# I2S9/dexterous-rl-manipulation

Measured on AMD Instinct MI355X. Metric: env-steps/sec @4096 envs/GPU, 1/2/4/8 MI355X; %HBM roofline step kernel, higher is better.
Workload: dtype bf16 MFMA (f32 acc) + f32/f64 env; 1 GPU; config_easy.json PG iteration: fused actor-MLP(256,256) rollout of 200 env steps x 4096 envs + critic fwd + GAE + adv-norm + PPO-clip / value heads + backward + Adam (1 epoch x 1 minibatch: ratio == 1, an A2C-style step); learner=pg, envs_per_gpu=4096, global_envs=4096, horizon=200, parallelism=dp1, world_size=1, ranks_per_gpu=1, overlap_comm=False, reserve_cus=0, reuse_h2=True

## Files before the change

### dexterous-rl-manipulation_amd/csrc/dxrl_mfma.h

```cpp
#pragma once
#include <hip/hip_runtime.h>
#include <stdint.h>

namespace dxrl {

typedef __bf16 bf16;
typedef bf16 bf16x8 __attribute__((ext_vector_type(8)));
typedef float f32x16 __attribute__((ext_vector_type(16)));
typedef bf16 bf16x4 __attribute__((ext_vector_type(4)));
typedef __attribute__((address_space(3))) bf16x4 lds_bf16x4;
typedef __attribute__((address_space(3))) bf16 lds_bf16;

__device__ __forceinline__ bf16x8 zero8() {
    bf16x8 z;
#pragma unroll
    for (int j = 0; j < 8; ++j) z[j] = (bf16)0.0f;
    return z;
}

__device__ __forceinline__ f32x16 mfma32(const bf16x8& a, const bf16x8& b, const f32x16& c) {
    return __builtin_amdgcn_mfma_f32_32x32x16_bf16(a, b, c, 0, 0, 0);
}

typedef float f32x4 __attribute__((ext_vector_type(4)));
__device__ __forceinline__ f32x4 mfma16(const bf16x8& a, const bf16x8& b, const f32x4& c) {
    return __builtin_amdgcn_mfma_f32_16x16x32_bf16(a, b, c, 0, 0, 0);
}

__device__ __forceinline__ bf16 to_bf16(float x) { return (bf16)x; }
__device__ __forceinline__ float from_bf16(bf16 x) { return (float)x; }

__device__ __forceinline__ int acc_row(int reg, int lane) { return (reg & 3) + 8 * (reg >> 2) + 4 * (lane >> 5); }

__device__ __forceinline__ bf16x8 load_frag(const bf16* base, int64_t ld, int64_t row, int64_t rows_valid, int k) {
    if (row < rows_valid) return *reinterpret_cast<const bf16x8*>(base + row * ld + k);
    bf16x8 z;
#pragma unroll
    for (int j = 0; j < 8; ++j) z[j] = (bf16)0.0f;
    return z;
}
// ... 71 lines not shown
```

### dexterous-rl-manipulation_amd/csrc/dxrl_pg_fused.hip

```cpp
#include "dxrl_gemm.h"
#include "dxrl_pg.h"

#include <stdio.h>
#include <stdlib.h>

#include <vector>

using namespace dxrl;
using namespace dxrl::pg;

namespace dxrl {
namespace {

constexpr float kLog2PiF = 1.8378770664093453f;
constexpr int kXp = kIn + 8;
constexpr int kHp = kH + 8;
constexpr int kDp = kOut + 8;

template <int kTR>
struct TileLds {
    static constexpr int kOffX = 0;
    static constexpr int kOffH1 = kOffX + kTR * kXp;
    static constexpr int kOffH2 = kOffH1 + kTR * kHp;
    static constexpr int kOffD = kOffH2 + kTR * kHp;
    static constexpr int kElems = kOffD + kTR * kDp;
    static_assert(kElems * 2 * (128 / kTR) == 163840, "one CU's 160 KiB of LDS per 128 samples");
};

// ... 16 lines not shown
    const bf16* X;
    const bf16 *W1, *W2, *W3, *W2T, *W3T;
    const bf16* W3rm;
    const float* b2;
    const float* b3;
    const float* logstd;
    const float* act;
    const float* logp_old;
    const float* adv;
    const float* ret;
    const double* stats;
    float sc, clip_eps, vf2;
    float* v_out;
    bf16* h1_out;
    bf16* dh2_out;
    const bf16* h2_in;
    bf16* h2_out;
    float* part;
    double* loss;
    int loss_rows;
    unsigned long long* stamps;
};

__device__ __forceinline__ void glds_x4(const void* src, const void* lds_dst) {
    const uint32_t lds_addr =
        __builtin_amdgcn_readfirstlane((uint32_t)(uintptr_t)(__attribute__((address_space(3))) const char*)lds_dst);
    uint32_t keep;
    asm volatile("s_mov_b32 %0, m0\n\ts_mov_b32 m0, %2\n\ts_nop 0\n\tglobal_load_lds_dwordx4 %1, off\n\ts_mov_b32 m0, %0"
                 : "=&s"(keep)
                 : "v"(src), "s"(lds_addr)
                 : "memory");
}

__device__ __forceinline__ void zero_acc(f32x16& a) {
#pragma unroll
    for (int q = 0; q < 16; ++q) a[q] = 0.0f;
}

struct NoHook {
    __device__ void operator()() const {}
};
struct NoKHook {
    __device__ void operator()(int) const {}
};
template <int KS>
struct WPre {
    static constexpr int kD = KS < 8 ? KS : 8;
    bf16x8 wf[kD];
    const gbf16x8* wp;
};
template <int KS>
__device__ __forceinline__ void w_prefetch(WPre<KS>& w, const bf16* W, int kst, int ft0, int lane) {
    w.wp = (const gbf16x8*)W + (int64_t)ft0 * kst * 64 + lane;
#pragma unroll
    for (int k = 0; k < WPre<KS>::kD; ++k) w.wf[k] = w.wp[64 * k];
}
template <int KS, int kLda, int MT, typename Hook = NoHook>
__device__ __forceinline__ void fwd_run(WPre<KS>& w, const bf16* A, f32x16 (&acc)[MT], int lane, Hook hook = Hook{},
                                        bool no_mfma = false) {
    const int r = lane & 31, h = lane >> 5;
    constexpr int kD = WPre<KS>::kD;
#pragma unroll
    for (int mt = 0; mt < MT; ++mt) zero_acc(acc[mt]);
    const bf16* ap = A + r * kLda + 8 * h;
    bf16x8 bq[2][MT];
#pragma unroll
    for (int mt = 0; mt < MT; ++mt) bq[0][mt] = *reinterpret_cast<const bf16x8*>(ap + 32 * mt * kLda);
#pragma unroll
    for (int k = 0; k < KS; ++k) {
        if (k + 1 < KS) {
#pragma unroll
            for (int mt = 0; mt < MT; ++mt)
                bq[(k + 1) & 1][mt] = *reinterpret_cast<const bf16x8*>(ap + 32 * mt * kLda + 16 * (k + 1));
        }
        const bf16x8 a = w.wf[k % kD];
        if (k + kD < KS) w.wf[k % kD] = w.wp[64 * (k + kD)];
        if (k + kD == KS) hook();
        __builtin_amdgcn_sched_barrier(0);
#pragma unroll
        for (int mt = 0; mt < MT; ++mt)
            if (!no_mfma) acc[mt] = mfma32(a, bq[k & 1][mt], acc[mt]);
        __builtin_amdgcn_sched_barrier(0);
    }
}
template <int KS, int kLda, int MT, typename Hook = NoHook>
__device__ __forceinline__ void fwd_tiles(const bf16* __restrict__ W, int kst, int ft0, const bf16* A,
                                          f32x16 (&acc)[MT], int lane, Hook hook = Hook{}, bool no_mfma = false) {
    WPre<KS> w;
    w_prefetch(w, W, kst, ft0, lane);
    fwd_run<KS, kLda, MT>(w, A, acc, lane, hook, no_mfma);
}

template <int KS, int kLda, int MT, typename Epi, typename KHook = NoKHook, typename THook = NoKHook>
__device__ __forceinline__ void fwd_pipe_w(const bf16x8 (&wf)[KS], const bf16* A, int lane, Epi& epi,
                                           bool no_mfma = false, KHook khook = KHook{}, THook thook = THook{}) {
    static_assert(KS >= 4 && KS % 4 == 0, "pair schedule assumes KS in {4, 8, 16, ...}");
    const int r = lane & 31, h = lane >> 5;
    constexpr int kPairsPerK = KS >= 8 ? 1 : 8 / KS;
    constexpr int kKPerPair = KS >= 8 ? KS / 8 : 1;
// ... 22 lines not shown
                for (int q = 0; q < kPairsPerK; ++q) epi(prev, mt - 1, (k / kKPerPair) * kPairsPerK + q);
            }
            khook(sidx);
            __builtin_amdgcn_sched_barrier(0);
        }
        prev = acc;
    }
    epi.prime(MT - 1);
#pragma unroll
    for (int q = 0; q < 8; ++q) {
        epi(prev, MT - 1, q);
        thook(q);
    }
}
template <int KS, int kLda, int MT, typename Epi, typename Hook = NoHook, typename KHook = NoKHook,
          typename THook = NoKHook>
__device__ __forceinline__ void fwd_pipe(WPre<KS>& w, const bf16* A, int lane, Epi& epi, Hook hook = Hook{},
                                         bool no_mfma = false, KHook khook = KHook{}, THook thook = THook{}) {
    constexpr int kD = WPre<KS>::kD;
    bf16x8 wf[KS];
#pragma unroll
    for (int k = 0; k < kD; ++k) wf[k] = w.wf[k];
#pragma unroll
    for (int k = kD; k < KS; ++k) wf[k] = w.wp[64 * k];
    hook();
    fwd_pipe_w<KS, kLda, MT>(wf, A, lane, epi, no_mfma, khook, thook);
}

struct EpiTanh {
    bf16* H;
    int f0;
    int r;
    const float* bk;
    bf16x4 v;
    __device__ void prime(int) {}
    __device__ __forceinline__ void operator()(const f32x16& acc, int mt, int p) {
        const int g = p >> 1, u = 2 * (p & 1);
        const f32x2 b = bk ? f32x2{bk[4 * g + u], bk[4 * g + u + 1]} : f32x2{0.0f, 0.0f};
        const f32x2 t = tanh_pre2(f32x2{acc[4 * g + u], acc[4 * g + u + 1]}, b);
        v[u] = to_bf16(t.x);
        v[u + 1] = to_bf16(t.y);
        if (u == 2) *reinterpret_cast<bf16x4*>(H + (32 * mt + r) * kHp + f0 + 8 * g) = v;
    }
};
struct EpiTanhB {
    bf16* H;
    int f0;
// ... 66 lines not shown
template <int MT>
__device__ __forceinline__ void gate_store(const f32x16 (&acc)[MT], const bf16x4 (&ys)[4][MT], int ft, bf16* Y,
                                           int lane) {
    const int r = lane & 31, h = lane >> 5;
#pragma unroll
    for (int g = 0; g < 4; ++g) {
        const int f0 = 32 * ft + 8 * g + 4 * h;
#pragma unroll
        for (int mt = 0; mt < MT; ++mt) {
            const bf16x4 y = ys[g][mt];
            bf16x4 v;
#pragma unroll
            for (int u = 0; u < 4; u += 2) {
                const f32x2 t = tanh_gate2(f32x2{acc[mt][4 * g + u], acc[mt][4 * g + u + 1]},
                                           f32x2{from_bf16(y[u]), from_bf16(y[u + 1])});
                v[u] = to_bf16(t.x);
                v[u + 1] = to_bf16(t.y);
            }
            *reinterpret_cast<bf16x4*>(Y + (32 * mt + r) * kHp + f0) = v;
        }
    }
}

template <int kThreads, int kTR>
__device__ __forceinline__ void copy_tile_out_n(const bf16* T, bf16* out, int64_t ld, int64_t m0, int64_t rows,
                                                int t, int diag) {
    constexpr int kChunks = kTR * (kH / 8);
    static_assert(kChunks % kThreads == 0, "whole chunks per thread");
    if (diag & 1) return;
    asm volatile("" : "+v"(t));
#pragma unroll
    for (int u = 0; u < kChunks / kThreads; ++u) {
        const int c = t + kThreads * u, row = c >> 5, col = 8 * (c & 31);
        const int64_t m = m0 + row;
        const bf16x8 v = *reinterpret_cast<const bf16x8*>(T + row * kHp + col);
        if (m < rows) *(__attribute__((address_space(1))) bf16x8*)(out + m * ld + col) = v;
    }
}

__device__ __forceinline__ void store_dh2(bf16* dst, const bf16x8& v) { *(__attribute__((address_space(1))) bf16x8*)dst = v; }

template <typename T>
__device__ __forceinline__ T* opaque(T* ptr) {
    asm volatile("" : "+s"(ptr));
    return ptr;
}

#ifndef DXRL_L2_PIPE
#define DXRL_L2_PIPE 1
#endif
#ifndef DXRL_DH2_IN_DH1
#define DXRL_DH2_IN_DH1 1
#endif
#ifndef DXRL_CRITIC_HEAD16
#define DXRL_CRITIC_HEAD16 1
#endif
#ifndef DXRL_ACTOR_HEAD16
#define DXRL_ACTOR_HEAD16 1
#endif
#ifndef DXRL_HEAD_PF
#define DXRL_HEAD_PF 1
#endif
#ifndef DXRL_FWD_RESIDENT_W
// ... 64 lines not shown
        for (int q = 0; q < 4; ++q) {
            acc3[j][0][q] = acc3[j][1][q] = 0.0f;
#pragma unroll
            for (int ri = 0; ri < 2; ++ri)
#pragma unroll
                for (int ci = 0; ci < 3; ++ci) acc1[j][ri][ci][q] = 0.0f;
        }
    float dls[8], db3[8];
#pragma unroll
    for (int j = 0; j < 8; ++j) dls[j] = db3[j] = 0.0f;
    float db2 = 0.0f;
    float lsum[4] = {0.0f, 0.0f, 0.0f, 0.0f};

    const auto uniform_f64 = [](double v) {
        const uint64_t u = __double_as_longlong(v);
        const uint32_t lo = __builtin_amdgcn_readfirstlane((uint32_t)u), hi = __builtin_amdgcn_readfirstlane((uint32_t)(u >> 32));
        return __longlong_as_double((long long)(((uint64_t)hi << 32) | lo));
    };
    const double adv_mean = uniform_f64(kTrain && actor ? p.stats[2] : 0.0);
    const double adv_inv = uniform_f64(kTrain && actor ? 1.0 / (p.stats[4] + 1e-8) : 1.0);

    constexpr int kXU = kTR * (kIn / 8) / kFThreads;
    bf16x8 xr[kXU];
    auto fetch_x = [&](int64_t tile) {
        int t = tid;
        asm volatile("" : "+v"(t));
#pragma unroll
        for (int u = 0; u < kXU; ++u) {
            const int c = t + kFThreads * u, row = c >> 3, col = 8 * (c & 7);
            const int64_t m = tile * kTR + row;
            xr[u] = m < p.rows ? *reinterpret_cast<const bf16x8*>(p.X + m * kIn + col) : zero8();
        }
    };
    unsigned long long st_acc[16], st_last = 0;
#pragma unroll
    for (int k = 0; k < 16; ++k) st_acc[k] = 0;
#define STAMP(k)                                                                                 \
    do {                                                                                         \
        if (diag & 8) {                                                                        \
            __builtin_amdgcn_sched_barrier(0);                                                   \
            unsigned long long t_;                                                               \
            asm volatile("s_memtime %0\n\ts_waitcnt lgkmcnt(0)" : "=s"(t_)::"memory");          \
            __builtin_amdgcn_sched_barrier(0);                                                   \
            st_acc[k] += t_ - st_last;                                                           \
            st_last = t_;                                                                        \
        }                                                                                        \
    } while (0)
    constexpr bool kResW = !kTrain && kNT == 1 && DXRL_FWD_RESIDENT_W && DXRL_L2_PIPE;
    constexpr bool kEarlyX = kResW && DXRL_FWD_EARLY_X;
    constexpr bool kResW1 = kResW || kH2;
    constexpr bool kDw1Tail = kTrain && kNT == 1 && kMT == 4 && DXRL_DW1_TAIL && DXRL_DH2_IN_DH1;
    bf16x8 w1res[kResW1 ? kIn / 16 : 1], w2res[kResW ? kH / 16 : 1];
    if constexpr (kResW1) {
        const gbf16x8* p1 = (const gbf16x8*)p.W1 + (int64_t)ft0 * (kIn / 16) * 64 + lane;
// ... 15 lines not shown
    float ahls[kResA ? 4 : 1], ahb3[kResA ? 4 : 1];
    if constexpr (kResA) {
#pragma unroll
        for (int i = 0; i < 4; ++i) {
            const int o = 4 * (lane >> 4) + i;
            ahls[i] = o < kAct ? ((gf32*)p.logstd)[o] : 0.0f;
            ahb3[i] = ((gf32*)p.b3)[(int64_t)o * kHx];
        }
    }
    if constexpr (kResB) {
        const int h0 = (threadIdx.x & 63) >> 5;
#pragma unroll
        for (int q = 0; q < 16; ++q)
            bkres[q] = tanh_bias(((gf32*)p.b2)[(int64_t)(32 * ft0 + 8 * (q >> 2) + 4 * h0 + (q & 3)) * kHx]);
    }
    if constexpr (kResH) {
        {
#pragma unroll
            for (int k = 0; k < 8; ++k)
                w3res[k] = (lane & 15) == 0 ? *(const gbf16x8*)(p.W3rm + 32 * k + 8 * (lane >> 4)) : zero8();
            b3res = ((gf32*)p.b3)[0];
        }
    }
    int64_t tile = blockIdx.x;
    if (tile < ntiles) fetch_x(tile);
    STAMP(15);
    for (; tile < ntiles; tile += gridDim.x) {
        const int64_t m0 = tile * kTR;
        int tid_l = (int)threadIdx.x;
        asm volatile("" : "+v"(tid_l));
        const int lane = tid_l & 63, r = lane & 31, h = lane >> 5;
        (void)r;
        (void)h;
        const bf16 *W1 = opaque(p.W1), *W2 = opaque(p.W2), *W3 = opaque(p.W3), *W2T = opaque(p.W2T),
                   *W3T = opaque(p.W3T);
        const float *b2 = opaque(p.b2), *b3 = opaque(p.b3), *logstd = opaque(p.logstd);
#pragma unroll
        for (int u = 0; u < kXU; ++u) {
            const int c = tid + kFThreads * u, row = c >> 3, col = 8 * (c & 7);
            *reinterpret_cast<bf16x8*>(X + row * kXp + col) = xr[u];
        }
        if constexpr (kEarlyX) {
            if (tile + gridDim.x < ntiles) fetch_x(tile + gridDim.x);
        }
        WPre<kIn / 16> pw1;
        if constexpr (kResW1) {
#pragma unroll
            for (int k = 0; k < kIn / 16; ++k) pw1.wf[k] = w1res[k];
        } else {
            w_prefetch(pw1, W1, kIn / 16, ft0, lane);
        }
        float hv2 = 0.0f, adv2 = 0.0f;
        float4 a02 = make_float4(0.f, 0.f, 0.f, 0.f);
        constexpr int kPieces = kTR * kHp * 2 / 1024;
        static_assert(kTR * kHp * 2 % 1024 == 0, "whole 1 KiB pieces");
        if constexpr (kH2) {
            const int64_t m16 = m0 + 16 * wave + (lane & 15), mc = m16 < p.rows ? m16 : p.rows - 1;
            if constexpr (kNet == 1) {
                hv2 = p.ret[mc];
            } else {
                hv2 = p.logp_old[mc];
                a02 = *reinterpret_cast<const float4*>(p.act + mc * kActPad + 4 * (lane >> 4));
                adv2 = p.adv[mc];
            }
        }
        const bool h2_issuer = kH2 && __builtin_amdgcn_readfirstlane(wave) >= kFW / 2;
        const auto h2_dma_k = [&](int sidx) {
            if constexpr (kH2) {
                if (sidx != 0 || !h2_issuer) return;
                const int64_t valid = (p.rows - m0 < kTR ? p.rows - m0 : kTR) * (int64_t)kHp * 2;
                const char* src = reinterpret_cast<const char*>(p.h2_in + m0 * kHp);
                char* dst = reinterpret_cast<char*>(H2);
                for (int q = __builtin_amdgcn_readfirstlane(wave) - kFW / 2; q < kPieces; q += kFW / 2) {
                    int64_t off = (int64_t)q * 1024 + 16 * lane;
                    off = off < valid ? off : valid - 16;
                    glds_x4(src + off, dst + q * 1024);
                }
            }
        };
        STAMP(0);
        __syncthreads();
        STAMP(1);

#pragma unroll 1
        for (int j = 0; j < kNT; ++j) {
            if (j > 0) w_prefetch(pw1, W1, kIn / 16, ft0 + j, lane);
            EpiTanh e1{H1, 32 * (ft0 + j) + 4 * h, r, nullptr};
            if constexpr (kH2) fwd_pipe<kIn / 16, kXp, kMT>(pw1, X, lane, e1, NoHook{}, false, h2_dma_k);
            else fwd_pipe<kIn / 16, kXp, kMT>(pw1, X, lane, e1);
        }
        WPre<kH / 16> pw2;
        if constexpr (!kResW && !kH2) w_prefetch(pw2, W2, kH / 16, ft0, lane);
        STAMP(2);
        if constexpr (!kH2) __syncthreads();
        STAMP(3);
        const int ml = 32 * wave + r;
        const int64_t m = m0 + ml;
        const bool valid = m < p.rows;
        float4 a0 = make_float4(0.f, 0.f, 0.f, 0.f), a1 = a0;
        float hv = 0.0f, adv = 0.0f;
        float bk[16];
        int bft = ft0;
        auto head_inputs = [&]() {
#pragma unroll
            for (int q = 0; q < 16; ++q) {
                if constexpr (kResB) bk[q] = bkres[q];
                else bk[q] = tanh_bias(((gf32*)b2)[(int64_t)(32 * bft + 8 * (q >> 2) + 4 * h + (q & 3)) * kHx]);
            }
            if constexpr (kCH16) {
                if (kTrain) {
                    const int64_t m16 = m0 + 16 * wave + (lane & 15);
                    hv = p.ret[m16 < p.rows ? m16 : p.rows - 1];
                }
                return;
            }
            if constexpr (kAH16) {
                const int64_t m16 = m0 + 16 * wave + (lane & 15), mc = m16 < p.rows ? m16 : p.rows - 1;
                hv = p.logp_old[mc];
                a0 = *reinterpret_cast<const float4*>(p.act + mc * kActPad + 4 * (lane >> 4));
                adv = p.adv[mc];
                return;
            }
            if (!kTrain || __builtin_amdgcn_readfirstlane(wave) >= kHW) return;
            const int64_t mc = valid ? m : p.rows - 1;
            hv = (actor ? p.logp_old : p.ret)[mc];
            if (actor) {
                a0 = *reinterpret_cast<const float4*>(p.act + mc * kActPad + 4 * h);
                a1 = *reinterpret_cast<const float4*>(p.act + mc * kActPad + 8 + 4 * h);
                adv = p.adv[mc];
            }
        };
#pragma unroll 1
        for (int j = 0; j < (kH2 ? 0 : kNT); ++j) {
            bft = ft0 + j;
            const auto l2_hook = [&]() {
                if (j == kNT - 1) head_inputs();
                else {
#pragma unroll
                    for (int q = 0; q < 16; ++q)
                        bk[q] = tanh_bias(((gf32*)b2)[(int64_t)(32 * bft + 8 * (q >> 2) + 4 * h + (q & 3)) * kHx]);
                }
            };
            if (j > 0) w_prefetch(pw2, W2, kH / 16, ft0 + j, lane);
#if DXRL_L2_PIPE
            EpiTanh e2{H2, 32 * (ft0 + j) + 4 * h, r, bk};
            if constexpr (kResW) {
                EpiTanh e2r{H2, 32 * (ft0 + j) + 4 * h, r, bkres};
                fwd_pipe_w<kH / 16, kHp, kMT>(w2res, H1, lane, e2r, (diag & 32) != 0);
            } else {
                fwd_pipe<kH / 16, kHp, kMT>(pw2, H1, lane, e2, l2_hook, (diag & 32) != 0);
            }
#else
            f32x16 acc[kMT];
            fwd_run<kH / 16, kHp, kMT>(pw2, H1, acc, lane, l2_hook, (diag & 32) != 0);
            if (!(diag & 16)) store_hidden(acc, ft0 + j, bk, H2, lane);
#endif
        }
        constexpr int kW3K = kH / 16;
        constexpr bool kHeadPf = kTrain && DXRL_HEAD_PF && kNet == 1;
        constexpr int kW3P = kTrain ? (kHeadPf ? kW3K / 2 : 1) : kW3K;
        bf16x8 w3p[kW3P];
        float b3p[8];
        const gbf16x8* w3row = (const gbf16x8*)W3 + lane;
        bf16x8 w3h[kH16 ? 8 : 1];
        float b3h = 0.0f;
        if constexpr (kAH16) {
            const bf16* W3rm = opaque(p.W3rm) + (lane & 15) * kHx + 8 * (lane >> 4);
#pragma unroll
            for (int k = 0; k < 8; ++k) w3h[k] = *(const gbf16x8*)(W3rm + 32 * k);
        }
        if constexpr (kResH) {
#pragma unroll
            for (int k = 0; k < 8; ++k) w3h[k] = w3res[k];
            b3h = b3res;
        } else if constexpr (kCH16) {
            const bf16* W3rm = opaque(p.W3rm);
#pragma unroll
            for (int k = 0; k < 8; ++k)
                w3h[k] = (lane & 15) == 0 ? *(const gbf16x8*)(W3rm + 32 * k + 8 * (lane >> 4)) : zero8();
            b3h = ((gf32*)b3)[0];
        }
        if (!kH16 && (!kTrain || kHeadPf)) {
            if (wave < kHW) {
#pragma unroll
                for (int k = 0; k < kW3P; ++k) w3p[k] = w3row[64 * k];
                if (kTrain) {
#pragma unroll
                    for (int q = 0; q < 8; ++q) b3p[q] = ((gf32*)b3)[(int64_t)((q & 3) + 8 * (q >> 2) + 4 * h) * kHx];
                }
            }
        }
        if constexpr (kH2) {
            hv = hv2;
            a0 = a02;
            adv = adv2;
            if (h2_issuer) __builtin_amdgcn_s_waitcnt(0xF70);
        }
        STAMP(4);
        __syncthreads();
        STAMP(5);

        if constexpr (kTrain && kFW > kHW && !kH16) {
            if (wave >= kHW && p.h1_out)
                copy_tile_out_n<64 * (kFW - kHW), kTR>(H1, p.h1_out, kHx, m0, p.rows, tid - 64 * kHW, diag);
        }
        if constexpr (kCH16) {
            const int s16 = 16 * wave + (lane & 15);
            const bf16* hb = H2 + s16 * kHp + 8 * (lane >> 4);
            f32x4 a16 = {0.0f, 0.0f, 0.0f, 0.0f};
#pragma unroll
            for (int k = 0; k < 8; ++k) a16 = mfma16(w3h[k], *reinterpret_cast<const bf16x8*>(hb + 32 * k), a16);
            const int64_t m16 = m0 + s16;
            const bool v16 = m16 < p.rows && lane < 16;
            const float v = a16[0] + b3h;
            float d0 = 0.0f;
            if (!kTrain) {
                if (v16) p.v_out[m16] = v;
            } else if (v16) {
                const float e = v - hv;
                d0 = from_bf16(to_bf16(p.vf2 * e * p.sc));
                db3[0] += d0;
                lsum[1] += e * e;
            }
            if (kTrain) {
                bf16x8 dv = zero8();
                if (lane < 16) dv[0] = to_bf16(d0);
                *reinterpret_cast<bf16x8*>(D + s16 * kDp + 8 * (lane >> 4)) = dv;
            }
        } else if constexpr (kAH16) {
            const int s16 = 16 * wave + (lane & 15), g4 = lane >> 4;
            const bf16* hb = H2 + s16 * kHp + 8 * g4;
            f32x4 a16 = {0.0f, 0.0f, 0.0f, 0.0f};
#pragma unroll
            for (int k = 0; k < 8; ++k) a16 = mfma16(w3h[k], *reinterpret_cast<const bf16x8*>(hb + 32 * k), a16);
            const int64_t m16 = m0 + s16;
            const bool v16 = m16 < p.rows;
            float mu[4], a[4], lsv[4], iv2[4], t[4], d[4];
            a[0] = a0.x; a[1] = a0.y; a[2] = a0.z; a[3] = a0.w;
#pragma unroll
            for (int i = 0; i < 4; ++i) {
                const int o = 4 * g4 + i;
                if constexpr (kResA) lsv[i] = ahls[i];
                else lsv[i] = o < kAct ? ((gf32*)logstd)[o] : 0.0f;
                iv2[i] = __expf(-2.0f * lsv[i]);
                if constexpr (kResA) mu[i] = a16[i] + ahb3[i];
                else mu[i] = a16[i] + ((gf32*)b3)[(int64_t)o * kHx];
                const float z = (a[i] - mu[i]) * __expf(-lsv[i]);
                t[i] = o < kAct ? -0.5f * z * z - lsv[i] - 0.5f * kLog2PiF : 0.0f;
                d[i] = 0.0f;
            }
            float tt[16];
#pragma unroll
            for (int g = 0; g < 4; ++g)
#pragma unroll
                for (int i = 0; i < 4; ++i) tt[4 * g + i] = __shfl(t[i], (lane & 15) + 16 * g);
            float lp = 0.0f;
#pragma unroll
            for (int o = 0; o < kAct; ++o) lp += tt[o];
            const float lo = hv;
// ... 138 lines not shown
            } else {
                const float v = acc[0] + b3v[0];
                if (!kTrain) {
                    if (valid && h == 0) p.v_out[m] = v;
                } else if (valid && h == 0) {
                    const float e = v - hv;
                    d[0] = from_bf16(to_bf16(p.vf2 * e * p.sc));
                    db3[0] += d[0];
                    lsum[1] += e * e;
                }
            }
            if (kTrain) {
#pragma unroll
                for (int g2 = 0; g2 < 4; ++g2) {
                    bf16x4 v;
#pragma unroll
                    for (int u = 0; u < 4; ++u) v[u] = g2 < 2 ? to_bf16(d[4 * g2 + u]) : (bf16)0.0f;
                    *reinterpret_cast<bf16x4*>(D + ml * kDp + 8 * g2 + 4 * h) = v;
                }
            }
        }
        STAMP(6);
        if (!kTrain) {
            if (p.h2_out) copy_tile_out_n<kFThreads, kTR>(H2, p.h2_out, kHp, m0, p.rows, tid, diag);
            if (!kEarlyX && tile + gridDim.x < ntiles) fetch_x(tile + gridDim.x);
            __syncthreads();
            STAMP(7);
            continue;
        }
        if constexpr (kFW == kHW || kH16) {
            if (p.h1_out) copy_tile_out_n<kFThreads, kTR>(H1, p.h1_out, kHx, m0, p.rows, tid, diag);
        }
        WPre<1> pw3t;
        w_prefetch(pw3t, W3T, kOut / 16, ft0, lane);
        STAMP(7);
        __syncthreads();
        STAMP(8);

#pragma unroll
        for (int kk = 0; kk < kTR; kk += 32) {
            const bf16x8 a = wg_frag<kDp>(D, 0, kk, lane);
#pragma unroll
            for (int j = 0; j < kNT; ++j)
#pragma unroll
                for (int ci = 0; ci < 2; ++ci)
                    if (!(diag & 4))
                        acc3[j][ci] = mfma16(a, wg_frag<kHp>(H2, 32 * (ft0 + j) + 16 * ci, kk, lane), acc3[j][ci]);
        }
#pragma unroll 1
        for (int j = 0; j < kNT; ++j) {
            f32x16 acc[kMT];
            bf16x4 ys[4][kMT];
            gate_load(ys, ft0 + j, H2, lane);
            if (j == 0) fwd_run<1, kDp, kMT>(pw3t, D, acc, lane);
// ... 17 lines not shown
#pragma unroll
            for (int rr = 0; rr < kRows; ++rr) {
                const bf16x4 v = rv[rr];
                cs.x += from_bf16(v[0]);
                cs.y += from_bf16(v[1]);
                cs.z += from_bf16(v[2]);
                cs.w += from_bf16(v[3]);
            }
            reinterpret_cast<float4*>(lds + kOffD)[wave * 64 + lane] = cs;
        }
#pragma unroll 1
        for (int j = 0; j < kNT; ++j) {
            if (j > 0) w_prefetch(pw2t, W2T, kH / 16, ft0 + j, lane);
            EpiGate eg{H1, 32 * (ft0 + j) + 4 * h, r};
#if DXRL_DH2_IN_DH1
            bf16x8 cv;
            const auto copy_k = [&](int sidx) {
                constexpr int kSteps = kMT * (kH / 16);
                constexpr int kFirst = (kSteps - kH / 16) / kCopyU >= 4 ? kH / 16 : 2;
                constexpr int kEvery = (kSteps - kFirst) / kCopyU, kAhead = kEvery >= 4 ? 3 : kEvery - 1;
                static_assert(kAhead >= 1 && kFirst >= kAhead && kFirst + kEvery * kCopyU <= kSteps, "copy schedule");
                if (diag & 1 || sidx < kFirst - kAhead) return;
                const int i = (sidx - (kFirst - kAhead)) / kEvery, ph = (sidx - (kFirst - kAhead)) % kEvery;
                const int c = tid_l + kFThreads * i, row = c >> 5, col = 8 * (c & 31);
                if (ph == 0 && i < kCopyU) cv = *reinterpret_cast<const bf16x8*>(H2 + row * kHp + col);
                if (ph == kAhead && i < kCopyU && m0 + row < p.rows) store_dh2(p.dh2_out + (m0 + row) * kH + col, cv);
            };
            if constexpr (kDw1Tail) {
                const auto dw1_tail = [&](int q) {
                    if (q != 1 && q != 3 && q != 5) return;
                    const int kk = 32 * (q >> 1);
                    if (kk == 0 && tile + gridDim.x < ntiles) fetch_x(tile + gridDim.x);
                    bf16x8 b[3];
#pragma unroll
                    for (int ci = 0; ci < 3; ++ci) b[ci] = wg_frag<kXp>(X, 16 * ci, kk, lane);
#pragma unroll
                    for (int ri = 0; ri < 2; ++ri) {
                        const bf16x8 a = wg_frag<kHp>(H1, 32 * ft0 + 16 * ri, kk, lane);
#pragma unroll
                        for (int ci = 0; ci < 3; ++ci)
                            if (!(diag & 4)) acc1[0][ri][ci] = mfma16(a, b[ci], acc1[0][ri][ci]);
                    }
                };
                fwd_pipe<kH / 16, kHp, kMT>(pw2t, H2, lane, eg, NoHook{}, false, copy_k, dw1_tail);
            } else {
                fwd_pipe<kH / 16, kHp, kMT>(pw2t, H2, lane, eg, NoHook{}, false, copy_k);
            }
#else
            fwd_pipe<kH / 16, kHp, kMT>(pw2t, H2, lane, eg);
#endif
        }
        STAMP(11);
        const auto db2_stage2 = [&]() {
            if (tid < kH) {
                const float* cs = reinterpret_cast<const float*>(lds + kOffD);
#pragma unroll
                for (int w = 0; w < kFW; ++w) db2 += cs[w * kH + tid_l];
            }
        };
        if constexpr (!kDw1Tail) {
            __syncthreads();
            STAMP(12);
            if (tile + gridDim.x < ntiles) fetch_x(tile + gridDim.x);
#if !DXRL_DH2_IN_DH1
            copy_tile_out_n<kFThreads, kTR>(H2, p.dh2_out, kH, m0, p.rows, tid, diag);
#endif
            db2_stage2();
        }
#pragma unroll
        for (int kk = kDw1Tail ? 96 : 0; kk < kTR; kk += 32) {
            bf16x8 b[3];
#pragma unroll
            for (int ci = 0; ci < 3; ++ci) b[ci] = wg_frag<kXp>(X, 16 * ci, kk, lane);
#pragma unroll
            for (int j = 0; j < kNT; ++j)
#pragma unroll
                for (int ri = 0; ri < 2; ++ri) {
                    const bf16x8 a = wg_frag<kHp>(H1, 32 * (ft0 + j) + 16 * ri, kk, lane);
#pragma unroll
                    for (int ci = 0; ci < 3; ++ci)
                        if (!(diag & 4)) acc1[j][ri][ci] = mfma16(a, b[ci], acc1[j][ri][ci]);
                }
        }
        STAMP(13);
        __syncthreads();
        STAMP(14);
        if constexpr (kDw1Tail) db2_stage2();
    }
    if ((diag & 8) && lane == 0) {
#pragma unroll
        for (int k = 0; k < 16; ++k) p.stamps[((int64_t)blockIdx.x * kFW + wave) * 16 + k] = st_acc[k];
    }
#undef STAMP
    if (!kTrain) return;

    float* part = p.part + (int64_t)blockIdx.x * kPartSize;
    {
        const int c16 = lane & 15, g16 = lane >> 4;
#pragma unroll
        for (int j = 0; j < kNT; ++j)
#pragma unroll
            for (int i = 0; i < 4; ++i) {
                const int o = 4 * g16 + i;
#pragma unroll
                for (int ci = 0; ci < 2; ++ci) part[kPartW3 + o * kPW3C + 32 * (ft0 + j) + 16 * ci + c16] = acc3[j][ci][i];
#pragma unroll
                for (int ri = 0; ri < 2; ++ri) {
                    float* row = part + kPartW1 + (32 * (ft0 + j) + 16 * ri + o) * kPW1C;
#pragma unroll
                    for (int ci = 0; ci < 3; ++ci) row[16 * ci + c16] = acc1[j][ri][ci][i];
// ... 151 lines not shown
__device__ __forceinline__ void fwd_pipe_w_mt(int mt, const bf16x8 (&wf)[KS], const bf16* A, int lane, Epi& epi) {
    switch (mt) {
        case 1: fwd_pipe_w<KS, kLda, 1>(wf, A, lane, epi); break;
        case 2: fwd_pipe_w<KS, kLda, 2>(wf, A, lane, epi); break;
        case 3: fwd_pipe_w<KS, kLda, 3>(wf, A, lane, epi); break;
        default: fwd_pipe_w<KS, kLda, 4>(wf, A, lane, epi); break;
    }
}
__global__ __launch_bounds__(512, 1) void k_pg_values(FusedArgs p) {
    using L = TileLds<128>;
    constexpr int kXU = 128 * (kIn / 8) / 512;
    __shared__ __attribute__((aligned(16))) bf16 lds[L::kElems];
    bf16* X = lds + L::kOffX;
    bf16* H1 = lds + L::kOffH1;
    bf16* H2 = lds + L::kOffH2;
    const int tid = threadIdx.x, lane = tid & 63, wave = tid >> 6, r = lane & 31, h = lane >> 5;
#if DXRL_FUSED_PRIO
    if (__builtin_amdgcn_readfirstlane(wave) >= 4) __builtin_amdgcn_s_setprio(1);
#endif
    const int64_t G = gridDim.x, b = blockIdx.x;
    const int64_t full = p.rows / 128 / G, main_rows = full * G * 128, rem = p.rows - main_rows;
    const int64_t rper = (rem + G - 1) / G;
    const int64_t r_lo = main_rows + b * rper, r_hi = min(p.rows, r_lo + rper);
    const int64_t ntile = full + (r_hi > r_lo ? 1 : 0);
    if (ntile == 0) return;
    const auto row0 = [&](int64_t k) { return k < full ? (b + k * G) * 128 : r_lo; };
    const auto count = [&](int64_t k) { return k < full ? (int64_t)128 : r_hi - r_lo; };
    bf16x8 xr[kXU];
    const auto fetch_x = [&](int64_t k) {
        const int64_t base = row0(k), cnt = count(k);
#pragma unroll
        for (int u = 0; u < kXU; ++u) {
            const int c = tid + 512 * u, row = c >> 3, col = 8 * (c & 7);
            xr[u] = row < cnt ? *reinterpret_cast<const bf16x8*>(p.X + (base + row) * kIn + col) : zero8();
        }
    };
    const auto store_x = [&]() {
#pragma unroll
        for (int u = 0; u < kXU; ++u) {
            const int c = tid + 512 * u, row = c >> 3, col = 8 * (c & 7);
            *reinterpret_cast<bf16x8*>(X + row * kXp + col) = xr[u];
        }
    };
    int64_t k = 0;
    fetch_x(k);
    bf16x8 w1[kIn / 16], w2[kH / 16], w3h[8];
    {
        const gbf16x8* p1 = (const gbf16x8*)p.W1 + (int64_t)wave * (kIn / 16) * 64 + lane;
#pragma unroll
        for (int q = 0; q < kIn / 16; ++q) w1[q] = p1[64 * q];
        const gbf16x8* p2 = (const gbf16x8*)p.W2 + (int64_t)wave * (kH / 16) * 64 + lane;
#pragma unroll
        for (int q = 0; q < kH / 16; ++q) w2[q] = p2[64 * q];
#pragma unroll
        for (int q = 0; q < 8; ++q)
            w3h[q] = (lane & 15) == 0 ? *(const gbf16x8*)(p.W3rm + 32 * q + 8 * (lane >> 4)) : zero8();
    }
    float bk[16];
#pragma unroll
    for (int q = 0; q < 16; ++q) bk[q] = tanh_bias(((gf32*)p.b2)[(int64_t)(32 * wave + 8 * (q >> 2) + 4 * h + (q & 3)) * kHx]);
    const float b3h = ((gf32*)p.b3)[0];
    EpiTanh e1{H1, 32 * wave + 4 * h, r, nullptr};
    EpiTanhB e2{H2, 32 * wave + 4 * h, r, {}, {}};
#pragma unroll
    for (int q = 0; q < 16; ++q) e2.bk[q] = bk[q];
    const auto mts = [&](int64_t kk) { return (int)((count(kk) + 31) / 32); };
    store_x();
    if (k + 1 < ntile) fetch_x(k + 1);
    __syncthreads();
    fwd_pipe_w_mt<kIn / 16, kXp>(mts(k), w1, X, lane, e1);
    __syncthreads();
    for (;;) {
        fwd_pipe_w_mt<kH / 16, kHp>(mts(k), w2, H1, lane, e2);
        if (k + 1 < ntile) {
            store_x();
            if (k + 2 < ntile) fetch_x(k + 2);
        }
        __syncthreads();
        if (p.h2_out) {
            const int64_t h2_m0 = row0(k), h2_end = row0(k) + count(k);
#pragma unroll
            for (int u = 0; u < 8; ++u) {
                const int c = tid + 512 * u, row = c >> 5, col = 8 * (c & 31);
                const bf16x8 v = *reinterpret_cast<const bf16x8*>(H2 + row * kHp + col);
                if (h2_m0 + row < h2_end)
                    __builtin_nontemporal_store(v, reinterpret_cast<bf16x8*>(p.h2_out + (h2_m0 + row) * kHp + col));
            }
        }
        const auto head = [&]() {
            const int s16 = 16 * wave + (lane & 15);
            if (s16 < 32 * mts(k)) {
                const bf16* hb = H2 + s16 * kHp + 8 * (lane >> 4);
                f32x4 a16 = {0.0f, 0.0f, 0.0f, 0.0f};
#pragma unroll
                for (int q = 0; q < 8; ++q) a16 = mfma16(w3h[q], *reinterpret_cast<const bf16x8*>(hb + 32 * q), a16);
                if (s16 < count(k) && lane < 16) p.v_out[row0(k) + s16] = a16[0] + b3h;
            }
        };
        if (k + 1 >= ntile) {
            head();
            break;
        }
        if (DXRL_VALUES_HEAD_SPLIT && __builtin_amdgcn_readfirstlane(wave) >= 4) {
            fwd_pipe_w_mt<kIn / 16, kXp>(mts(k + 1), w1, X, lane, e1);
            head();
        } else {
            head();
            fwd_pipe_w_mt<kIn / 16, kXp>(mts(k + 1), w1, X, lane, e1);
        }
        __syncthreads();
        ++k;
    }
}

__device__ __forceinline__ double fused_reduce_block(const float4* __restrict__ partial, int z, float* __restrict__ gW1,
                                                     float* __restrict__ gW3, float* __restrict__ gLs,
                                                     float* __restrict__ gW2, float ent_coef, int64_t blk,
                                                     float4 (*grp)[16]) {
    constexpr int kRX = 16;
// ... 229 lines not shown
                       gnorm_partial);
    return launch_check("k_grad_reduce_nets");
}

int dxrl_pg_gnorm_blocks(int32_t* blocks) {
    DXRL_REQUIRE(blocks, "null output");
    *blocks = (int32_t)(2 * ((kPartSize / 4 + 15) / 16 + kH * kH / 4 / 16));
    return DXRL_OK;
}

}

namespace dxrl {
namespace {
int fused_kernel(const dxrl_pg_fused_args* a, hipStream_t st, int* grid_out) {
    const bool train = a->train != 0;
    const bf16* w = static_cast<const bf16*>(a->packed);
    const bool c = a->net == 1;
    const int64_t o2 = c ? kOffW2c : kOffW2a, o3 = c ? kOffW3c : kOffW3a;
    FusedArgs f{};
    f.net = a->net;
    f.train = train;
    f.rows = a->rows;
    f.X = static_cast<const bf16*>(a->obs);
    const bf16* fr = w + kFr + (c ? kFrNet : 0);
    f.W1 = fr + kFrOffW1;
    f.W2 = fr + kFrOffW2;
    f.W3 = fr + kFrOffW3;
    f.W2T = fr + kFrOffW2T;
    f.W3T = fr + kFrOffW3T;
    f.W3rm = w + (c ? kBfW3c : kBfW3a);
    f.b2 = a->params + o2 + kH;
    f.b3 = a->params + o3 + kH;
    f.logstd = a->params + kOffLogStd;
    f.act = a->act;
    f.logp_old = a->logp_old;
    f.adv = a->adv;
    f.ret = a->ret;
    f.stats = a->stats;
    f.sc = (float)a->inv_total_samples;
    f.clip_eps = (float)a->clip_eps;
    f.vf2 = (float)(2.0 * a->vf_coef);
    f.v_out = a->values;
    const bool recompute = train && a->rows % 32 == 0 && a->h1_mode == 0;
    f.h1_out = recompute ? nullptr : static_cast<bf16*>(a->h1);
    f.dh2_out = static_cast<bf16*>(a->dh2);
// ... 70 lines not shown
```

Before: 501.4 million env-steps/s.

## Use scalar-base plus 32-bit lane offsets and split full and ragged tiles

Global loads and stores in the fused PG kernels now use an SGPR base pointer with a 32-bit per-lane VGPR offset instead of full 64-bit per-lane addresses. The per-tile loop is split into a full-tile specialization, which drops row bounds checks, and a single ragged tail tile. The goal is fewer 64-bit VALU address computations and fewer VGPRs, which may improve scheduling or occupancy. The cost is more template instantiations and code size, plus a new row-count limit check.

Result: no change. 504.6 million env-steps/s (median of 3 runs) (+0.6%).

```diff
diff --git a/dexterous-rl-manipulation_amd/csrc/dxrl_mfma.h b/dexterous-rl-manipulation_amd/csrc/dxrl_mfma.h
--- a/dexterous-rl-manipulation_amd/csrc/dxrl_mfma.h
+++ b/dexterous-rl-manipulation_amd/csrc/dxrl_mfma.h
@@ -16,6 +16,28 @@
 #pragma unroll
     for (int j = 0; j < 8; ++j) z[j] = (bf16)0.0f;
     return z;
+}
+
+typedef __attribute__((address_space(1))) char gchar;
+__device__ __forceinline__ const gchar* sbase(const gchar* p) {
+    asm volatile("" : "+s"(p));
+    return p;
+}
+__device__ __forceinline__ gchar* sbase(gchar* p) {
+    asm volatile("" : "+s"(p));
+    return p;
+}
+__device__ __forceinline__ int lane_off(int v) {
+    asm volatile("" : "+v"(v));
+    return v;
+}
+template <typename T>
+__device__ __forceinline__ T gld(const gchar* base, uint32_t off) {
+    return *(const __attribute__((address_space(1))) T*)(base + off);
+}
+template <typename T>
+__device__ __forceinline__ void gst(gchar* base, uint32_t off, const T& v) {
+    *(__attribute__((address_space(1))) T*)(base + off) = v;
 }
 
 __device__ __forceinline__ f32x16 mfma32(const bf16x8& a, const bf16x8& b, const f32x16& c) {
diff --git a/dexterous-rl-manipulation_amd/csrc/dxrl_pg_fused.hip b/dexterous-rl-manipulation_amd/csrc/dxrl_pg_fused.hip
--- a/dexterous-rl-manipulation_amd/csrc/dxrl_pg_fused.hip
+++ b/dexterous-rl-manipulation_amd/csrc/dxrl_pg_fused.hip
@@ -4,6 +4,7 @@
 #include <stdio.h>
 #include <stdlib.h>
 
+#include <type_traits>
 #include <vector>
 
 using namespace dxrl;
@@ -66,13 +67,13 @@
     unsigned long long* stamps;
 };
 
-__device__ __forceinline__ void glds_x4(const void* src, const void* lds_dst) {
+__device__ __forceinline__ void glds_x4(const gchar* base, uint32_t off, const void* lds_dst) {
     const uint32_t lds_addr =
         __builtin_amdgcn_readfirstlane((uint32_t)(uintptr_t)(__attribute__((address_space(3))) const char*)lds_dst);
     uint32_t keep;
-    asm volatile("s_mov_b32 %0, m0\n\ts_mov_b32 m0, %2\n\ts_nop 0\n\tglobal_load_lds_dwordx4 %1, off\n\ts_mov_b32 m0, %0"
+    asm volatile("s_mov_b32 %0, m0\n\ts_mov_b32 m0, %3\n\ts_nop 0\n\tglobal_load_lds_dwordx4 %1, %2\n\ts_mov_b32 m0, %0"
                  : "=&s"(keep)
-                 : "v"(src), "s"(lds_addr)
+                 : "v"(off), "s"(base), "s"(lds_addr)
                  : "memory");
 }
 
@@ -91,13 +92,16 @@
 struct WPre {
     static constexpr int kD = KS < 8 ? KS : 8;
     bf16x8 wf[kD];
-    const gbf16x8* wp;
+    const gchar* wb;
+    uint32_t lo;
+    __device__ __forceinline__ bf16x8 frag(int k) const { return gld<bf16x8>(sbase(wb + 4096 * (k / 4)) + 1024 * (k % 4), lo); }
 };
 template <int KS>
 __device__ __forceinline__ void w_prefetch(WPre<KS>& w, const bf16* W, int kst, int ft0, int lane) {
-    w.wp = (const gbf16x8*)W + (int64_t)ft0 * kst * 64 + lane;
-#pragma unroll
-    for (int k = 0; k < WPre<KS>::kD; ++k) w.wf[k] = w.wp[64 * k];
+    w.wb = (const gchar*)W + (int64_t)__builtin_amdgcn_readfirstlane(ft0) * kst * 1024;
+    w.lo = 16 * lane_off(lane);
+#pragma unroll
+    for (int k = 0; k < WPre<KS>::kD; ++k) w.wf[k] = w.frag(k);
 }
 template <int KS, int kLda, int MT, typename Hook = NoHook>
 __device__ __forceinline__ void fwd_run(WPre<KS>& w, const bf16* A, f32x16 (&acc)[MT], int lane, Hook hook = Hook{},
@@ -118,7 +122,7 @@
                 bq[(k + 1) & 1][mt] = *reinterpret_cast<const bf16x8*>(ap + 32 * mt * kLda + 16 * (k + 1));
         }
         const bf16x8 a = w.wf[k % kD];
-        if (k + kD < KS) w.wf[k % kD] = w.wp[64 * (k + kD)];
+        if (k + kD < KS) w.wf[k % kD] = w.frag(k + kD);
         if (k + kD == KS) hook();
         __builtin_amdgcn_sched_barrier(0);
 #pragma unroll
@@ -187,7 +191,7 @@
 #pragma unroll
     for (int k = 0; k < kD; ++k) wf[k] = w.wf[k];
 #pragma unroll
-    for (int k = kD; k < KS; ++k) wf[k] = w.wp[64 * k];
+    for (int k = kD; k < KS; ++k) wf[k] = w.frag(k);
     hook();
     fwd_pipe_w<KS, kLda, MT>(wf, A, lane, epi, no_mfma, khook, thook);
 }
@@ -300,23 +304,24 @@
     }
 }
 
-template <int kThreads, int kTR>
-__device__ __forceinline__ void copy_tile_out_n(const bf16* T, bf16* out, int64_t ld, int64_t m0, int64_t rows,
-                                                int t, int diag) {
+template <int kThreads, int kTR, bool kFull, int kLd>
+__device__ __forceinline__ void copy_tile_out_n(const bf16* T, bf16* out, int64_t m0, int cnt, int t, int diag) {
     constexpr int kChunks = kTR * (kH / 8);
     static_assert(kChunks % kThreads == 0, "whole chunks per thread");
+    static_assert((int64_t)kTR * kLd * 2 < (int64_t)1 << 31, "tile-relative byte offsets fit 32 bits");
     if (diag & 1) return;
     asm volatile("" : "+v"(t));
+    static_assert(kThreads % 32 == 0, "a thread's chunks share a column");
+    gchar* ob = (gchar*)out + m0 * (kLd * 2);
+    const int row0 = t >> 5, col = 8 * (t & 31);
 #pragma unroll
     for (int u = 0; u < kChunks / kThreads; ++u) {
-        const int c = t + kThreads * u, row = c >> 5, col = 8 * (c & 31);
-        const int64_t m = m0 + row;
+        const int row = row0 + (kThreads / 32) * u;
         const bf16x8 v = *reinterpret_cast<const bf16x8*>(T + row * kHp + col);
-        if (m < rows) *(__attribute__((address_space(1))) bf16x8*)(out + m * ld + col) = v;
-    }
-}
-
-__device__ __forceinline__ void store_dh2(bf16* dst, const bf16x8& v) { *(__attribute__((address_space(1))) bf16x8*)dst = v; }
+        if (kFull || row < cnt) gst(sbase(ob + (kThreads / 32) * u * kLd * 2), (uint32_t)(row0 * kLd + col) * 2, v);
+    }
+}
+
 
 template <typename T>
 __device__ __forceinline__ T* opaque(T* ptr) {
@@ -427,14 +432,16 @@
 
     constexpr int kXU = kTR * (kIn / 8) / kFThreads;
     bf16x8 xr[kXU];
-    auto fetch_x = [&](int64_t tile) {
+    auto fetch_x = [&](auto full, int64_t tile) __attribute__((always_inline)) {
+        constexpr bool kFull = decltype(full)::value;
         int t = tid;
         asm volatile("" : "+v"(t));
+        const gchar* xb = (const gchar*)p.X + tile * (kTR * kIn * 2);
+        const int cnt = kFull ? kTR : (int)(p.rows - tile * kTR);
 #pragma unroll
         for (int u = 0; u < kXU; ++u) {
-            const int c = t + kFThreads * u, row = c >> 3, col = 8 * (c & 7);
-            const int64_t m = tile * kTR + row;
-            xr[u] = m < p.rows ? *reinterpret_cast<const bf16x8*>(p.X + m * kIn + col) : zero8();
+            const int row = (t >> 3) + (kFThreads / 8) * u;
+            xr[u] = kFull || row < cnt ? gld<bf16x8>(sbase(xb + 16 * kFThreads * u), 16u * t) : zero8();
         }
     };
     unsigned long long st_acc[16], st_last = 0;
@@ -496,11 +503,21 @@
             b3res = ((gf32*)p.b3)[0];
         }
     }
-    int64_t tile = blockIdx.x;
-    if (tile < ntiles) fetch_x(tile);
-    STAMP(15);
-    for (; tile < ntiles; tile += gridDim.x) {
+    static_assert((int64_t)kTR * (kHx * 2 > kActPad * 4 ? kHx * 2 : kActPad * 4) < (int64_t)1 << 31,
+                  "tile-relative byte offsets fit 32 bits");
+    const int64_t nfull = p.rows / kTR;
+    constexpr std::true_type kFullTile{};
+    constexpr std::false_type kRaggedTile{};
+    const auto tile_body = [&](auto full, const int64_t tile, const bool more_full) __attribute__((always_inline)) {
+        constexpr bool kFull = decltype(full)::value;
         const int64_t m0 = tile * kTR;
+        const int cnt = kFull ? kTR : (int)(p.rows - m0);
+        (void)cnt;
+        const auto fetch_next_x = [&]() __attribute__((always_inline)) {
+            if constexpr (kFull) {
+                if (more_full) fetch_x(kFullTile, tile + gridDim.x);
+            }
+        };
         int tid_l = (int)threadIdx.x;
         asm volatile("" : "+v"(tid_l));
         const int lane = tid_l & 63, r = lane & 31, h = lane >> 5;
@@ -511,12 +528,10 @@
         const float *b2 = opaque(p.b2), *b3 = opaque(p.b3), *logstd = opaque(p.logstd);
 #pragma unroll
         for (int u = 0; u < kXU; ++u) {
-            const int c = tid + kFThreads * u, row = c >> 3, col = 8 * (c & 7);
+            const int row = (tid >> 3) + (kFThreads / 8) * u, col = 8 * (tid & 7);
             *reinterpret_cast<bf16x8*>(X + row * kXp + col) = xr[u];
         }
-        if constexpr (kEarlyX) {
-            if (tile + gridDim.x < ntiles) fetch_x(tile + gridDim.x);
-        }
+        if constexpr (kEarlyX) fetch_next_x();
         WPre<kIn / 16> pw1;
         if constexpr (kResW1) {
 #pragma unroll
@@ -528,27 +543,38 @@
         float4 a02 = make_float4(0.f, 0.f, 0.f, 0.f);
         constexpr int kPieces = kTR * kHp * 2 / 1024;
         static_assert(kTR * kHp * 2 % 1024 == 0, "whole 1 KiB pieces");
+        const auto head_row = [&]() __attribute__((always_inline)) {
+            const int s16 = 16 * wave + (lane & 15);
+            return (uint32_t)(kFull || s16 < cnt ? s16 : cnt - 1);
+        };
+        const auto head_in_critic = [&](float& hv_) __attribute__((always_inline)) {
+            hv_ = gld<float>((const gchar*)p.ret + m0 * 4, 4 * head_row());
+        };
+        const auto head_in_actor = [&](float& hv_, float4& a_, float& adv_) __attribute__((always_inline)) {
+            const uint32_t s = head_row();
+            hv_ = gld<float>((const gchar*)p.logp_old + m0 * 4, 4 * s);
+            const f32x4 av = gld<f32x4>((const gchar*)p.act + m0 * (kActPad * 4), (s * kActPad + 4 * (lane >> 4)) * 4);
+            a_ = make_float4(av[0], av[1], av[2], av[3]);
+            adv_ = gld<float>((const gchar*)p.adv + m0 * 4, 4 * s);
+        };
         if constexpr (kH2) {
-            const int64_t m16 = m0 + 16 * wave + (lane & 15), mc = m16 < p.rows ? m16 : p.rows - 1;
-            if constexpr (kNet == 1) {
-                hv2 = p.ret[mc];
-            } else {
-                hv2 = p.logp_old[mc];
-                a02 = *reinterpret_cast<const float4*>(p.act + mc * kActPad + 4 * (lane >> 4));
-                adv2 = p.adv[mc];
-            }
+            if constexpr (kNet == 1) head_in_critic(hv2);
+            else head_in_actor(hv2, a02, adv2);
         }
         const bool h2_issuer = kH2 && __builtin_amdgcn_readfirstlane(wave) >= kFW / 2;
         const auto h2_dma_k = [&](int sidx) {
             if constexpr (kH2) {
                 if (sidx != 0 || !h2_issuer) return;
-                const int64_t valid = (p.rows - m0 < kTR ? p.rows - m0 : kTR) * (int64_t)kHp * 2;
-                const char* src = reinterpret_cast<const char*>(p.h2_in + m0 * kHp);
+                const gchar* src = (const gchar*)p.h2_in + m0 * (kHp * 2);
                 char* dst = reinterpret_cast<char*>(H2);
+                const uint32_t valid = (uint32_t)cnt * (kHp * 2);
                 for (int q = __builtin_amdgcn_readfirstlane(wave) - kFW / 2; q < kPieces; q += kFW / 2) {
-                    int64_t off = (int64_t)q * 1024 + 16 * lane;
-                    off = off < valid ? off : valid - 16;
-                    glds_x4(src + off, dst + q * 1024);
+                    if constexpr (kFull) {
+                        glds_x4(src + q * 1024, 16u * lane, dst + q * 1024);
+                    } else {
+                        const uint32_t off = (uint32_t)q * 1024 + 16 * lane;
+                        glds_x4(src, off < valid ? off : valid - 16, dst + q * 1024);
+                    }
                 }
             }
         };
@@ -582,17 +608,11 @@
                 else bk[q] = tanh_bias(((gf32*)b2)[(int64_t)(32 * bft + 8 * (q >> 2) + 4 * h + (q & 3)) * kHx]);
             }
             if constexpr (kCH16) {
-                if (kTrain) {
-                    const int64_t m16 = m0 + 16 * wave + (lane & 15);
-                    hv = p.ret[m16 < p.rows ? m16 : p.rows - 1];
-                }
+                if (kTrain) head_in_critic(hv);
                 return;
             }
             if constexpr (kAH16) {
-                const int64_t m16 = m0 + 16 * wave + (lane & 15), mc = m16 < p.rows ? m16 : p.rows - 1;
-                hv = p.logp_old[mc];
-                a0 = *reinterpret_cast<const float4*>(p.act + mc * kActPad + 4 * (lane >> 4));
-                adv = p.adv[mc];
+                head_in_actor(hv, a0, adv);
                 return;
             }
             if (!kTrain || __builtin_amdgcn_readfirstlane(wave) >= kHW) return;
@@ -639,9 +659,10 @@
         bf16x8 w3h[kH16 ? 8 : 1];
         float b3h = 0.0f;
         if constexpr (kAH16) {
-            const bf16* W3rm = opaque(p.W3rm) + (lane & 15) * kHx + 8 * (lane >> 4);
-#pragma unroll
-            for (int k = 0; k < 8; ++k) w3h[k] = *(const gbf16x8*)(W3rm + 32 * k);
+            const gchar* W3rm = (const gchar*)opaque(p.W3rm);
+            const uint32_t wo = ((lane & 15) * kHx + 8 * (lane >> 4)) * 2;
+#pragma unroll
+            for (int k = 0; k < 8; ++k) w3h[k] = gld<bf16x8>(W3rm + 64 * k, wo);
         }
         if constexpr (kResH) {
 #pragma unroll
@@ -676,7 +697,7 @@
 
         if constexpr (kTrain && kFW > kHW && !kH16) {
             if (wave >= kHW && p.h1_out)
-                copy_tile_out_n<64 * (kFW - kHW), kTR>(H1, p.h1_out, kHx, m0, p.rows, tid - 64 * kHW, diag);
+                copy_tile_out_n<64 * (kFW - kHW), kTR, kFull, kHx>(H1, p.h1_out, m0, cnt, tid - 64 * kHW, diag);
         }
         if constexpr (kCH16) {
             const int s16 = 16 * wave + (lane & 15);
@@ -685,7 +706,7 @@
 #pragma unroll
             for (int k = 0; k < 8; ++k) a16 = mfma16(w3h[k], *reinterpret_cast<const bf16x8*>(hb + 32 * k), a16);
             const int64_t m16 = m0 + s16;
-            const bool v16 = m16 < p.rows && lane < 16;
+            const bool v16 = (kFull || s16 < cnt) && lane < 16;
             const float v = a16[0] + b3h;
             float d0 = 0.0f;
             if (!kTrain) {
@@ -707,8 +728,7 @@
             f32x4 a16 = {0.0f, 0.0f, 0.0f, 0.0f};
 #pragma unroll
             for (int k = 0; k < 8; ++k) a16 = mfma16(w3h[k], *reinterpret_cast<const bf16x8*>(hb + 32 * k), a16);
-            const int64_t m16 = m0 + s16;
-            const bool v16 = m16 < p.rows;
+            const bool v16 = kFull || s16 < cnt;
             float mu[4], a[4], lsv[4], iv2[4], t[4], d[4];
             a[0] = a0.x; a[1] = a0.y; a[2] = a0.z; a[3] = a0.w;
 #pragma unroll
@@ -893,14 +913,14 @@
         }
         STAMP(6);
         if (!kTrain) {
-            if (p.h2_out) copy_tile_out_n<kFThreads, kTR>(H2, p.h2_out, kHp, m0, p.rows, tid, diag);
-            if (!kEarlyX && tile + gridDim.x < ntiles) fetch_x(tile + gridDim.x);
+            if (p.h2_out) copy_tile_out_n<kFThreads, kTR, kFull, kHp>(H2, p.h2_out, m0, cnt, tid, diag);
+            if (!kEarlyX) fetch_next_x();
             __syncthreads();
             STAMP(7);
-            continue;
+            return;
         }
         if constexpr (kFW == kHW || kH16) {
-            if (p.h1_out) copy_tile_out_n<kFThreads, kTR>(H1, p.h1_out, kHx, m0, p.rows, tid, diag);
+            if (p.h1_out) copy_tile_out_n<kFThreads, kTR, kFull, kHx>(H1, p.h1_out, m0, cnt, tid, diag);
         }
         WPre<1> pw3t;
         w_prefetch(pw3t, W3T, kOut / 16, ft0, lane);
@@ -964,15 +984,16 @@
                 static_assert(kAhead >= 1 && kFirst >= kAhead && kFirst + kEvery * kCopyU <= kSteps, "copy schedule");
                 if (diag & 1 || sidx < kFirst - kAhead) return;
                 const int i = (sidx - (kFirst - kAhead)) / kEvery, ph = (sidx - (kFirst - kAhead)) % kEvery;
-                const int c = tid_l + kFThreads * i, row = c >> 5, col = 8 * (c & 31);
+                const int row = (tid_l >> 5) + (kFThreads / 32) * i, col = 8 * (tid_l & 31);
                 if (ph == 0 && i < kCopyU) cv = *reinterpret_cast<const bf16x8*>(H2 + row * kHp + col);
-                if (ph == kAhead && i < kCopyU && m0 + row < p.rows) store_dh2(p.dh2_out + (m0 + row) * kH + col, cv);
+                if (ph == kAhead && i < kCopyU && (kFull || row < cnt))
+                    gst(sbase((gchar*)p.dh2_out + m0 * (kH * 2) + 16 * kFThreads * i), 16u * tid_l, cv);
             };
             if constexpr (kDw1Tail) {
                 const auto dw1_tail = [&](int q) {
                     if (q != 1 && q != 3 && q != 5) return;
                     const int kk = 32 * (q >> 1);
-                    if (kk == 0 && tile + gridDim.x < ntiles) fetch_x(tile + gridDim.x);
+                    if (kk == 0) fetch_next_x();
                     bf16x8 b[3];
 #pragma unroll
                     for (int ci = 0; ci < 3; ++ci) b[ci] = wg_frag<kXp>(X, 16 * ci, kk, lane);
@@ -1003,9 +1024,9 @@
         if constexpr (!kDw1Tail) {
             __syncthreads();
             STAMP(12);
-            if (tile + gridDim.x < ntiles) fetch_x(tile + gridDim.x);
+            fetch_next_x();
 #if !DXRL_DH2_IN_DH1
-            copy_tile_out_n<kFThreads, kTR>(H2, p.dh2_out, kH, m0, p.rows, tid, diag);
+            copy_tile_out_n<kFThreads, kTR, kFull, kH>(H2, p.dh2_out, m0, cnt, tid, diag);
 #endif
             db2_stage2();
         }
@@ -1028,6 +1049,16 @@
         __syncthreads();
         STAMP(14);
         if constexpr (kDw1Tail) db2_stage2();
+    };
+    int64_t tile = blockIdx.x;
+    if (tile < nfull) fetch_x(kFullTile, tile);
+    else if (tile < ntiles) fetch_x(kRaggedTile, tile);
+    STAMP(15);
+    const int nmine = tile < nfull ? (int)((nfull - tile + gridDim.x - 1) / gridDim.x) : 0;
+    for (int it = 0; it < nmine; ++it, tile += gridDim.x) tile_body(kFullTile, tile, it + 1 < nmine);
+    if (tile < ntiles) {
+        if (nmine > 0) fetch_x(kRaggedTile, tile);
+        tile_body(kRaggedTile, tile, false);
     }
     if ((diag & 8) && lane == 0) {
 #pragma unroll
@@ -1225,27 +1256,32 @@
     const int64_t full = p.rows / 128 / G, main_rows = full * G * 128, rem = p.rows - main_rows;
     const int64_t rper = (rem + G - 1) / G;
     const int64_t r_lo = main_rows + b * rper, r_hi = min(p.rows, r_lo + rper);
-    const int64_t ntile = full + (r_hi > r_lo ? 1 : 0);
-    if (ntile == 0) return;
-    const auto row0 = [&](int64_t k) { return k < full ? (b + k * G) * 128 : r_lo; };
-    const auto count = [&](int64_t k) { return k < full ? (int64_t)128 : r_hi - r_lo; };
+    const int64_t ntile64 = full + (r_hi > r_lo ? 1 : 0);
+    if (ntile64 == 0) return;
+    const int nfull = (int)full, ntile = (int)ntile64, rcnt = (int)(r_hi - r_lo);
+    const auto row0 = [&](int k) { return k < nfull ? (b + k * G) * 128 : r_lo; };
+    const auto count = [&](int k) { return k < nfull ? 128 : rcnt; };
     bf16x8 xr[kXU];
-    const auto fetch_x = [&](int64_t k) {
-        const int64_t base = row0(k), cnt = count(k);
-#pragma unroll
-        for (int u = 0; u < kXU; ++u) {
-            const int c = tid + 512 * u, row = c >> 3, col = 8 * (c & 7);
-            xr[u] = row < cnt ? *reinterpret_cast<const bf16x8*>(p.X + (base + row) * kIn + col) : zero8();
+    const auto fetch_x = [&](int k) {
+        const gchar* xb = (const gchar*)p.X + row0(k) * (kIn * 2);
+        if (k < nfull) {
+            const uint32_t xo = 16u * lane_off(tid);
+#pragma unroll
+            for (int u = 0; u < kXU; ++u) xr[u] = gld<bf16x8>(sbase(xb + 8192 * u), xo);
+        } else {
+#pragma unroll
+            for (int u = 0; u < kXU; ++u)
+                xr[u] = (tid >> 3) + 64 * u < rcnt ? gld<bf16x8>(sbase(xb + 8192 * u), 16u * lane_off(tid)) : zero8();
         }
     };
     const auto store_x = [&]() {
 #pragma unroll
         for (int u = 0; u < kXU; ++u) {
-            const int c = tid + 512 * u, row = c >> 3, col = 8 * (c & 7);
+            const int row = (tid >> 3) + 64 * u, col = 8 * (tid & 7);
             *reinterpret_cast<bf16x8*>(X + row * kXp + col) = xr[u];
         }
     };
-    int64_t k = 0;
+    int k = 0;
     fetch_x(k);
     bf16x8 w1[kIn / 16], w2[kH / 16], w3h[8];
     {
@@ -1267,7 +1303,7 @@
     EpiTanhB e2{H2, 32 * wave + 4 * h, r, {}, {}};
 #pragma unroll
     for (int q = 0; q < 16; ++q) e2.bk[q] = bk[q];
-    const auto mts = [&](int64_t kk) { return (int)((count(kk) + 31) / 32); };
+    const auto mts = [&](int kk) { return (count(kk) + 31) / 32; };
     store_x();
     if (k + 1 < ntile) fetch_x(k + 1);
     __syncthreads();
@@ -1281,13 +1317,24 @@
         }
         __syncthreads();
         if (p.h2_out) {
-            const int64_t h2_m0 = row0(k), h2_end = row0(k) + count(k);
-#pragma unroll
-            for (int u = 0; u < 8; ++u) {
-                const int c = tid + 512 * u, row = c >> 5, col = 8 * (c & 31);
-                const bf16x8 v = *reinterpret_cast<const bf16x8*>(H2 + row * kHp + col);
-                if (h2_m0 + row < h2_end)
-                    __builtin_nontemporal_store(v, reinterpret_cast<bf16x8*>(p.h2_out + (h2_m0 + row) * kHp + col));
+            gchar* hb = (gchar*)p.h2_out + row0(k) * (kHp * 2);
+            const int hrow = tid >> 5, hcol = 8 * (tid & 31);
+            typedef __attribute__((address_space(1))) bf16x8 gbf16x8s;
+            if (k < nfull) {
+                const uint32_t ho = (uint32_t)lane_off(hrow * kHp + hcol) * 2;
+#pragma unroll
+                for (int u = 0; u < 8; ++u) {
+                    const bf16x8 v = *reinterpret_cast<const bf16x8*>(H2 + (hrow + 16 * u) * kHp + hcol);
+                    __builtin_nontemporal_store(v, (gbf16x8s*)(sbase(hb + 16 * u * kHp * 2) + ho));
+                }
+            } else {
+#pragma unroll
+                for (int u = 0; u < 8; ++u) {
+                    const bf16x8 v = *reinterpret_cast<const bf16x8*>(H2 + (hrow + 16 * u) * kHp + hcol);
+                    if (hrow + 16 * u < rcnt)
+                        __builtin_nontemporal_store(v, (gbf16x8s*)(sbase(hb + 16 * u * kHp * 2) +
+                                                                    (uint32_t)lane_off(hrow * kHp + hcol) * 2));
+                }
             }
         }
         const auto head = [&]() {
@@ -1297,7 +1344,7 @@
                 f32x4 a16 = {0.0f, 0.0f, 0.0f, 0.0f};
 #pragma unroll
                 for (int q = 0; q < 8; ++q) a16 = mfma16(w3h[q], *reinterpret_cast<const bf16x8*>(hb + 32 * q), a16);
-                if (s16 < count(k) && lane < 16) p.v_out[row0(k) + s16] = a16[0] + b3h;
+                if (s16 < count(k) && lane < 16) gst((gchar*)p.v_out + row0(k) * 4, 4u * lane_off(s16), a16[0] + b3h);
             }
         };
         if (k + 1 >= ntile) {
@@ -1573,6 +1620,7 @@
     f.net = a->net;
     f.train = train;
     f.rows = a->rows;
+    DXRL_REQUIRE(a->rows < ((int64_t)1 << 38), "fused: rows out of range");
     f.X = static_cast<const bf16*>(a->obs);
     const bf16* fr = w + kFr + (c ? kFrNet : 0);
     f.W1 = fr + kFrOffW1;
```
